# a1q123456/image_stitching

Hardware: AMD Instinct MI355X
Metric: 4K frames stitched/sec (higher is better)
Workload: dtype u8

## Files before the change

### image_stitching_amd/csrc/homography.h

```cpp
#pragma once
#include "common.h"

struct HomoCall {
    const float* src;
    const float* dst;
    uint8_t* mask;
    long long pt_off;
    int n;
    int active;
};

struct HomoResult {
    double H[9];
    int ok;
    int iters;
    int ninl;
    int pad;
};

struct HomoBatch {
    int count = 0;
    long long points = 0;
    int max_iters = 0;
    void* mem = nullptr;
    size_t bytes = 0;
    HomoCall* calls = nullptr;
    HomoResult* results = nullptr;
    void* state = nullptr;
    int* sub_idx = nullptr;
    double* Hc = nullptr;
    int* valid = nullptr;
    int* good = nullptr;
    float* scr = nullptr;
    double* rec = nullptr;
    unsigned* draw_next = nullptr;
    int* draw_idx = nullptr;
    int* fin = nullptr;
};

int homo_batch_reserve(MisContext* ctx, HomoBatch* b, int count, long long points, int max_iters);
int homo_batch_debug_states(MisContext* ctx, const HomoBatch* b, int* out, int cap);
void homo_batch_release(HomoBatch* b);
enum HomoRun {
    HOMO_BOTH_PHASES = 2,
    HOMO_PHASE0_REPLAY = 3,
    HOMO_PHASE1_REPLAY = 6,
    HOMO_TAIL0_MASK = 10,
    HOMO_TAIL0_REFINE = 11,
    HOMO_TAIL1_MASK = 12,
    HOMO_TAIL1_REFINE = 13,
};
struct HomoSync { hipEvent_t rec = nullptr; int rec_pos = 0; };
int homo_batch_run(MisContext* ctx, HomoBatch* b, double thresh, int max_iters, double confidence, HomoRun run = HOMO_BOTH_PHASES,
                   hipStream_t stream = nullptr, const HomoSync* sync = nullptr);
```

### image_stitching_amd/csrc/homography.hip

```cpp
#include "homography.h"
#include "dev_math.h"
#include <algorithm>
#include <mutex>
#include <vector>

namespace {

#ifndef MIS_PHASE0
#define MIS_PHASE0 128
#endif
constexpr int PHASE0 = MIS_PHASE0;
constexpr int RNG_TABLE = 1 << 17;
constexpr int TB = 256;

struct RansacState {
    int mode;
    int n_sub;
    int iter, niters, max_good, done, best_k, result;
    int tail_pending;
    int draw_k, draw_fail;
    long long draw_pos;
};

__device__ __forceinline__ bool jd_mid(int hi_word) { return (((unsigned)hi_word >> 20) & 0x7ffu) - 653u <= 740u; }
__device__ __forceinline__ double jd_div(double n, double d) {
    double r = __builtin_amdgcn_rcp(d);
    double e = __builtin_fma(-d, r, 1.0);
    r = __builtin_fma(r, e, r);
    e = __builtin_fma(-d, r, 1.0);
    r = __builtin_fma(r, e, r);
    const double q = n * r;
    e = __builtin_fma(-d, q, n);
    return __builtin_fma(e, r, q);
}
__device__ __forceinline__ double jd_sqrt_1to2(double x) {
    const double y = __builtin_amdgcn_rsq(x);
    double g = x * y, h = y * 0.5;
    const double r = __builtin_fma(-h, g, 0.5);
    g = __builtin_fma(g, r, g); h = __builtin_fma(h, r, h);
    double d = __builtin_fma(-g, g, x);
    g = __builtin_fma(d, h, g);
    d = __builtin_fma(-g, g, x);
    return __builtin_fma(d, h, g);
}
__device__ __forceinline__ double cv_hypot(double a, double b) {
    a = fabs(a); b = fabs(b);
    if (a > b) { b /= a; return a * sqrt(1 + b * b); }
    if (b > 0) { a /= b; return b * sqrt(1 + a * a); }
    return 0;
}
template <bool LEAN>
__device__ __forceinline__ void jacobi_rotation(double p, double y, double* c_, double* s_, double* t_) {
    double tt, sn, c;
    if (LEAN) {
        const double ap = fabs(p), ay = fabs(y);
        const double big = fmax(ap, ay), q1 = jd_div(fmin(ap, ay), big);
        tt = ay + big * jd_sqrt_1to2(1 + q1 * q1);
        const double q2 = jd_div(ap, tt);
        sn = tt * jd_sqrt_1to2(1 + q2 * q2);
        c = jd_div(tt, sn);
        sn = jd_div(p, sn); tt = jd_div(p, tt) * p;
    } else {
        tt = fabs(y) + cv_hypot(p, y);
        sn = cv_hypot(p, tt);
        c = tt / sn;
// ... 98 lines not shown
    if (d.lds_mod && rel >= 0 && rel < d.lds_n) return (int)d.lds_u[rel];
    return (int)(draw_at(d, pos) % (unsigned)n);
}

__device__ __forceinline__ long long attempt_len(DrawCtx& d, long long pos, int n, int* idx) {
    for (int i = 0; i < 4; i++) {
        int idx_i;
        bool dup;
        do {
            idx_i = draw_mod_at(d, pos++, n);
            dup = false;
            for (int q = 0; q < i; q++) dup |= idx[q] == idx_i;
        } while (dup);
        idx[i] = idx_i;
    }
    return pos;
}
__device__ __forceinline__ bool subset_passes(const float* src, const float* dst, const int* idx) {
    float ms1[8], ms2[8];
    for (int i = 0; i < 4; i++) {
        const float2 ps = reinterpret_cast<const float2*>(src)[idx[i]], pd = reinterpret_cast<const float2*>(dst)[idx[i]];
        ms1[2 * i] = ps.x; ms1[2 * i + 1] = ps.y;
        ms2[2 * i] = pd.x; ms2[2 * i + 1] = pd.y;
    }
    return check_subset(ms1, ms2);
}

__device__ long long attempt_at(DrawCtx& d, long long pos, const float* src, const float* dst, int n, int* idx, bool* pass) {
    float ms1[8], ms2[8];
    for (int i = 0; i < 4; i++) {
        int idx_i;
        bool dup;
        do {
            idx_i = (int)(draw_at(d, pos++) % (unsigned)n);
            dup = false;
            for (int q = 0; q < i; q++) dup |= idx[q] == idx_i;
        } while (dup);
        idx[i] = idx_i;
        const float2 ps = reinterpret_cast<const float2*>(src)[idx_i], pd = reinterpret_cast<const float2*>(dst)[idx_i];
        ms1[2 * i] = ps.x; ms1[2 * i + 1] = ps.y;
        ms2[2 * i] = pd.x; ms2[2 * i + 1] = pd.y;
    }
    *pass = check_subset(ms1, ms2);
    return pos;
}

constexpr int DRAW_CHUNK = 4096;
#ifndef MIS_DRAW_TB
#define MIS_DRAW_TB 1024
#endif
constexpr int DRAW_TB = MIS_DRAW_TB;
constexpr int DRAW_PTS = 2048;
__global__ __launch_bounds__(DRAW_TB) void draw_kernel(const HomoCall* calls, RansacState* states, int* sub_idx, int* draw_idx, const unsigned* U,
                                                  unsigned long long state_T, int max_iters, int phase, int k_hi_arg) {
#if MIS_CHAIN_PRIO
    __builtin_amdgcn_s_setprio(MIS_CHAIN_PRIO);
#endif
    __shared__ unsigned char tab[DRAW_CHUNK];
    __shared__ float2 pts[2 * DRAW_PTS];
    __shared__ long long s_pos;
    __shared__ int s_k, s_attempts, s_more, s_kfirst, s_nacc;
    __shared__ unsigned short acc_o[DRAW_CHUNK / 4];
    __shared__ unsigned short nxtA[DRAW_CHUNK + 1], nxtB[DRAW_CHUNK + 1];
    __shared__ unsigned char reach[DRAW_CHUNK];
    __shared__ unsigned su[DRAW_CHUNK + 128];
    __shared__ int scan[DRAW_TB];
    __shared__ int s_big, s_firstvis, s_lastaccvis;
    __shared__ long long s_endpos;
    const int b = blockIdx.x, t = threadIdx.x;
#ifdef MIS_TAIL_PROF
    const unsigned long long dpk = wall_clock64();
#endif
    const HomoCall c = calls[b];
    RansacState* st = states + b;
    if (phase == 0) {
        if (t == 0) {
            st->mode = (!c.active || c.n < 4) ? 0 : (c.n == 4 ? 1 : 2);
            st->n_sub = 0; st->iter = 0; st->niters = max_iters > 1 ? max_iters : 1; st->max_good = 0; st->done = 0; st->best_k = -1; st->result = 0; st->tail_pending = 0;
            st->draw_k = 0; st->draw_fail = 0; st->draw_pos = 0;
        }
        if (!c.active || c.n <= 4) return;
    } else {
        if (st->mode != 2 || st->done || st->draw_fail) return;
    }
    __syncthreads();
    const int k_hi = min(k_hi_arg, phase == 0 ? max_iters : st->niters);
    if (t == 0) { s_pos = st->draw_pos; s_k = st->draw_k; s_attempts = 0; s_more = s_k < k_hi; }
    __syncthreads();
    DrawCtx d;
    d.U = U; d.state_T = state_T; d.cur_state = state_T; d.cur_pos = RNG_TABLE;
    const float* psrc = c.src;
    const float* pdst = c.dst;
    if (c.n <= DRAW_PTS) {
        for (int i = t; i < c.n; i += DRAW_TB) { pts[i] = reinterpret_cast<const float2*>(c.src)[i]; pts[DRAW_PTS + i] = reinterpret_cast<const float2*>(c.dst)[i]; }
        psrc = reinterpret_cast<const float*>(pts); pdst = reinterpret_cast<const float*>(pts + DRAW_PTS);
        __syncthreads();
    }
    int* didx = draw_idx + (size_t)b * DRAW_CHUNK * 4;
    int* sidx = sub_idx + (size_t)b * max_iters * 4;
    if (phase == 0 && c.n <= 10) {
        const int n = c.n, total = n * (n - 1) * (n - 2) * (n - 3);
        int any = 0;
        for (int q = t; q < total && !any; q += DRAW_TB) {
            int r = q, id[4];
            id[0] = r % n; r /= n;
            int a1 = r % (n - 1); r /= (n - 1);
            int a2 = r % (n - 2); r /= (n - 2);
// ... 129 lines not shown
#ifdef MIS_TAIL_PROF
            dp_last = wall_clock64();
#endif
            continue;
        }
        __syncthreads();
        for (int o = t; o < DRAW_CHUNK; o += DRAW_TB) {
            if ((tab[o] & 0x7f) == 127) continue;
            int idx[4];
            attempt_len(d, base + o, c.n, idx);
            if (subset_passes(psrc, pdst, idx)) tab[o] |= 0x80;
            *reinterpret_cast<int4*>(didx + 4 * o) = make_int4(idx[0], idx[1], idx[2], idx[3]);
        }
        __syncthreads();
        if (t == 0) {
            long long pos = base;
            int k = s_k, attempts = s_attempts, nacc = 0;
            bool fail = false;
            while (k < k_hi && pos < base + DRAW_CHUNK) {
                unsigned char e = tab[pos - base];
                bool pass;
                if ((e & 0x7f) != 127) {
                    pass = (e & 0x80) != 0;
                    if (pass) acc_o[nacc++] = (unsigned short)(pos - base);
                    pos += e & 0x7f;
                } else {
                    int idx[4];
                    pos = attempt_at(d, pos, psrc, pdst, c.n, idx, &pass);
                    if (pass) { acc_o[nacc++] = 0xffff; sidx[4 * k] = idx[0]; sidx[4 * k + 1] = idx[1]; sidx[4 * k + 2] = idx[2]; sidx[4 * k + 3] = idx[3]; }
                }
                attempts++;
                if (pass) { k++; attempts = 0; }
                else if (attempts >= 10000) { fail = true; break; }
            }
            s_kfirst = s_k; s_nacc = nacc;
            s_pos = pos; s_k = k; s_attempts = attempts;
            s_more = !fail && k < k_hi;
            if (!s_more) { st->draw_pos = pos; st->draw_k = k; st->draw_fail = fail; st->n_sub = k; }
        }
        __syncthreads();
        for (int j = t; j < s_nacc; j += DRAW_TB) {
            const unsigned o = acc_o[j];
            if (o != 0xffff) *reinterpret_cast<int4*>(sidx + 4 * (s_kfirst + j)) = *reinterpret_cast<const int4*>(didx + 4 * o);
        }
        __syncthreads();
    }
#ifdef MIS_TAIL_PROF
    if (t == 0 && dp_chunks) {
        const int ph = phase ? 4 : 0;
        atomicAdd(&g_draw_prof[ph], (unsigned long long)dp_chunks); atomicMax(&g_draw_prof[ph + 1], (unsigned long long)dp_chunks);
        atomicMax(&g_draw_prof[ph + 2], wall_clock64() - dp0); atomicAdd(&g_draw_prof[ph + 3], 1ull);
    }
#endif
}

#ifdef MIS_TAIL_PROF
__device__ unsigned long long g_hyp_prof[8];
#endif
#ifndef MIS_HQ_HYPS
#define MIS_HQ_HYPS 64
#endif
constexpr int HQ_HYPS = MIS_HQ_HYPS;
constexpr int HQ_STRIDE = HQ_HYPS + 1;
constexpr int HQ_ELEMS = 127;
struct QSlot {
    double* base;
    __device__ __forceinline__ double& e(int idx) const { return base[idx * HQ_STRIDE]; }
};
__device__ __forceinline__ int hq_T(int r) { return ((r * (17 - r)) >> 1) - r - 1; }
constexpr int HQ_W = 36, HQ_V = 45, HQ_DUMMY = 126;

struct QCand { double a; int pk; };
template <int CTRL>
__device__ __forceinline__ QCand hq_step(const QCand& c) {
    const int hi = __builtin_amdgcn_update_dpp(0, __double2hiint(c.a), CTRL, 0xf, 0xf, false);
    const int lo = __builtin_amdgcn_update_dpp(0, __double2loint(c.a), CTRL, 0xf, 0xf, false);
    const int pk = __builtin_amdgcn_update_dpp(0, c.pk, CTRL, 0xf, 0xf, false);
    const double oa = __hiloint2double(hi, lo);
    const bool take = (c.a < oa) | ((c.a == oa) & (pk < c.pk));
    QCand r;
    r.a = take ? oa : c.a; r.pk = take ? pk : c.pk;
    return r;
}
__device__ __forceinline__ QCand hq_quad_best(QCand c) {
    c = hq_step<0xB1>(c);
    c = hq_step<0x4E>(c);
    return c;
}

__device__ void jacobi9_quad(const QSlot s, const int q) {
    constexpr int n = 9;
    const double eps = DBL_EPSILON;
    int ii[3];
    bool own[3];
#pragma unroll
    for (int j = 0; j < 3; j++) { ii[j] = q + 4 * j; own[j] = ii[j] < n; }
    for (int e = q; e < n * n; e += 4) s.e(HQ_V + e) = (e % (n + 1) == 0) ? 1. : 0.;
    __builtin_amdgcn_fence(__ATOMIC_ACQ_REL, "wavefront");
    int ir[3], ic[3];
    double arv[3], acv[3];
#pragma unroll
    for (int j = 0; j < 3; j++) {
        const int i = ii[j];
        ir[j] = 0; ic[j] = 0; arv[j] = -1.; acv[j] = -1.;
        if (own[j] && i < n - 1) {
            int m = i + 1;
            double mv = fabs(s.e(hq_T(i) + m));
            for (int c = i + 2; c < n; c++) { const double v = fabs(s.e(hq_T(i) + c)); if (mv < v) mv = v, m = c; }
            ir[j] = m; arv[j] = mv;
        }
        if (own[j] && i > 0) {
            int m = 0;
            double mv = fabs(s.e(hq_T(0) + i));
            for (int r = 1; r < i; r++) { const double v = fabs(s.e(hq_T(r) + i)); if (mv < v) mv = v, m = r; }
            ic[j] = m; acv[j] = mv;
// ... 87 lines not shown
            double tw = s.e(HQ_W + m); s.e(HQ_W + m) = s.e(HQ_W + k); s.e(HQ_W + k) = tw;
            for (int i = 0; i < n; i++) { double tv = s.e(HQ_V + n * m + i); s.e(HQ_V + n * m + i) = s.e(HQ_V + n * k + i); s.e(HQ_V + n * k + i) = tv; }
        }
        __builtin_amdgcn_fence(__ATOMIC_ACQ_REL, "wavefront");
    }
}

__device__ int dlt4_quad(const float* M, const float* m, const QSlot s, const int q, double* H) {
    const int count = 4;
    double cMx = 0, cMy = 0, cmx = 0, cmy = 0, sMx = 0, sMy = 0, smx = 0, smy = 0;
    for (int i = 0; i < count; i++) { cmx += m[2 * i]; cmy += m[2 * i + 1]; cMx += M[2 * i]; cMy += M[2 * i + 1]; }
    cmx /= count; cmy /= count; cMx /= count; cMy /= count;
    for (int i = 0; i < count; i++) {
        smx += fabs(m[2 * i] - cmx); smy += fabs(m[2 * i + 1] - cmy);
        sMx += fabs(M[2 * i] - cMx); sMy += fabs(M[2 * i + 1] - cMy);
    }
    if (fabs(smx) < DBL_EPSILON || fabs(smy) < DBL_EPSILON || fabs(sMx) < DBL_EPSILON || fabs(sMy) < DBL_EPSILON) return 0;
    smx = count / smx; smy = count / smy; sMx = count / sMx; sMy = count / sMy;
    double LtL[45];
#pragma unroll
    for (int e = 0; e < 45; e++) LtL[e] = 0;
#pragma unroll
    for (int i = 0; i < count; i++) {
        const double x = (m[2 * i] - cmx) * smx, y = (m[2 * i + 1] - cmy) * smy;
        const double X = (M[2 * i] - cMx) * sMx, Y = (M[2 * i + 1] - cMy) * sMy;
        const double Lx[9] = {X, Y, 1, 0, 0, 0, -x * X, -x * Y, -x};
        const double Ly[9] = {0, 0, 0, X, Y, 1, -y * X, -y * Y, -y};
        int e = 0;
#pragma unroll
        for (int j = 0; j < 9; j++)
#pragma unroll
            for (int k = j; k < 9; k++, e++) LtL[e] += Lx[j] * Lx[k] + Ly[j] * Ly[k];
    }
    {
        int e = 0;
#pragma unroll
        for (int j = 0; j < 9; j++)
#pragma unroll
            for (int k = j; k < 9; k++, e++) {
                if ((e & 3) != q) continue;
                if (k == j) s.e(HQ_W + j) = LtL[e];
                else s.e(hq_T(j) + k) = LtL[e];
            }
    }
    __builtin_amdgcn_fence(__ATOMIC_ACQ_REL, "wavefront");
    jacobi9_quad(s, q);
    double H0[9];
    for (int i = 0; i < 9; i++) H0[i] = s.e(HQ_V + 72 + i);
    const double nrm[8] = {cmx, cmy, cMx, cMy, smx, smy, sMx, sMy};
    dlt_denormalise(H0, nrm, H);
    return 1;
}

__global__ __launch_bounds__(4 * HQ_HYPS) void hyp_quad_kernel(const HomoCall* calls, const RansacState* states, const int* sub_idx, double* Hc, int* valid, int lo,
                                                               int max_iters) {
#if MIS_CHAIN_PRIO
    __builtin_amdgcn_s_setprio(MIS_CHAIN_PRIO);
#endif
    extern __shared__ double sl[];
    const int b = blockIdx.y, t = threadIdx.x, h = t >> 2, q = t & 3;
    const RansacState st = states[b];
    if (st.mode != 2 || st.done) return;
    const int limit = min(st.n_sub, st.niters);
    const int k = lo + blockIdx.x * HQ_HYPS + h;
    if (k >= limit) return;
    const HomoCall c = calls[b];
    const int* id = sub_idx + ((size_t)b * max_iters + k) * 4;
    float ms1[8], ms2[8];
#pragma unroll
    for (int i = 0; i < 4; i++) {
        int qq = id[i];
        ms1[2 * i] = c.src[2 * qq]; ms1[2 * i + 1] = c.src[2 * qq + 1];
        ms2[2 * i] = c.dst[2 * qq]; ms2[2 * i + 1] = c.dst[2 * qq + 1];
    }
    double H[9];
    const QSlot s{sl + h};
    const int ok = dlt4_quad(ms1, ms2, s, q, H);
    if (q == 0) {
        if (ok) {
            double* o = Hc + ((size_t)b * max_iters + k) * 9;
#pragma unroll
            for (int i = 0; i < 9; i++) o[i] = H[i];
        }
        valid[(size_t)b * max_iters + k] = ok;
    }
}

__global__ __launch_bounds__(256) void hyp_count_kernel(const HomoCall* calls, const RansacState* states, const double* Hc, const int* valid, int* good, int lo,
                                                        int max_iters, float thr) {
    const int b = blockIdx.y, lane = threadIdx.x & 63;
    const RansacState st = states[b];
    if (st.mode != 2 || st.done) return;
    const int limit = min(st.n_sub, st.niters);
    const int k = lo + blockIdx.x * 4 + (int)(threadIdx.x >> 6);
    if (k >= limit) return;
    const size_t e = (size_t)b * max_iters + k;
    int cnt = 0;
    if (valid[e]) {
        const HomoCall c = calls[b];
        float Hf[9];
#pragma unroll
        for (int i = 0; i < 9; i++) Hf[i] = (float)Hc[e * 9 + i];
        for (int i0 = 0; i0 < c.n; i0 += 64) {
            const int i = i0 + lane;
            const int f = i < c.n ? is_inlier(Hf, c.src[2 * i], c.src[2 * i + 1], c.dst[2 * i], c.dst[2 * i + 1], thr) : 0;
            cnt += __popcll(__ballot(f));
        }
    }
    if (lane == 0) good[e] = cnt;
}

#ifdef MIS_TAIL_PROF
__device__ unsigned long long g_jac_prof[8];
#ifdef MIS_JAC_PROF
#define JP_T(v) const unsigned long long v = __builtin_readcyclecounter()
#define JP_ADD(i, a, b) do { if (threadIdx.x == 0) atomicAdd(&g_jac_prof[i], (b) - (a)); } while (0)
#else
#define JP_T(v)
#define JP_ADD(i, a, b)
#endif
__device__ unsigned long long g_tail_log[6 * 1024];
__device__ unsigned g_tail_log_n;
__device__ unsigned long long g_tail_prof[12];
#define PROF_T0(v) unsigned long long v = wall_clock64()
#define PROF_ADD(i, v) do { if (threadIdx.x == 0) atomicAdd(&g_tail_prof[i], wall_clock64() - (v)); } while (0)
#define PROF_INC(i, n) do { if (threadIdx.x == 0) atomicAdd(&g_tail_prof[i], (unsigned long long)(n)); } while (0)
#else
#define PROF_T0(v)
#define PROF_ADD(i, v)
#define PROF_INC(i, n)
#define JP_T(v)
#define JP_ADD(i, a, b)
#endif
#ifndef MIS_PS_PTS
#define MIS_PS_PTS 32
#endif
constexpr int PS_PTS = MIS_PS_PTS;
constexpr int PS_TERMS = 42;
constexpr int PS_PITCH = 43;
constexpr int PS_STAGE = PS_PTS * PS_PITCH;
constexpr size_t TAIL_DYN_LDS = sizeof(double) * 2 * PS_STAGE;
struct TailShared {
    double A[81], V[81], W[9];
    double best[9], nrm[8];
    double lm[8 + 8 + 64 + 64 + 8 + 8 + 8 + 8];
    float Hf[9];
    int indR[9], indC[9];
    int np, go;
    int bad;
    double chunk[TB * 10];
    int staged;
#ifdef MIS_TAIL_PROF
    int prof_rot, prof_lm;
#endif
};
__device__ __forceinline__ float4 tail_load_point(const float* s1, const float* d1, int i) {
    const float2 dd = reinterpret_cast<const float2*>(d1)[i], ss = reinterpret_cast<const float2*>(s1)[i];
    return make_float4(dd.x, dd.y, ss.x, ss.y);
}
__device__ __forceinline__ void lds_barrier() { mis_lds_barrier(); }

__device__ __forceinline__ void wave_sync() {
// ... 520 lines not shown
        }
        __syncthreads();
        if (sc[6] != 0.) {
            if (t < 64) S.A[t] = A[t];
            __syncthreads();
            jacobi_eigen_coop<8>(S);
            if (t == 0) {
                double thrw = 0;
                for (int i = 0; i < 8; i++) thrw += S.W[i];
                thrw *= DBL_EPSILON * 2;
                for (int e = 0; e < 64; e++) Ap[e] = 0;
                for (int i = 0; i < 8; i++) {
                    double wi = S.W[i];
                    if (fabs(wi) <= thrw) continue;
                    wi = 1 / wi;
                    for (int r = 0; r < 8; r++)
                        for (int c = 0; c < 8; c++) Ap[r * 8 + c] = Ap[r * 8 + c] + S.V[i * 8 + r] * (S.V[i * 8 + c] * wi);
                }
                double maxval = DBL_EPSILON;
                for (int i = 0; i < 8; i++) { double a = fabs(Ap[i * 8 + i]); if (a > maxval) maxval = a; }
                double lambda = 1. / maxval, nu = sc[7] * 0.5;
                sc[5] = lambda;
                sc[4] = lambda * nu;
            }
            __syncthreads();
        }
        if (t == 0) {
            double Sv = sc[0], Sd = sc[1];
            sc[3] = Sd < Sv ? 1. : 0.;
            if (Sd < Sv) { sc[0] = Sd; for (int i = 0; i < 8; i++) x[i] = xd[i]; }
        }
        __syncthreads();
        if (sc[3] != 0.) normal_eq(x, true);
        iter++;
        PROF_INC(3, 1);
#ifdef MIS_TAIL_PROF
        if (t == 0) S.prof_lm++;
#endif
        double dmax = 0;
        for (int i = 0; i < 8; i++) { double a = fabs(d[i]); if (a > dmax) dmax = a; }
        bool proceed = iter < 10 && dmax >= (double)FLT_EPSILON && sc[2] >= (double)FLT_EPSILON;
        __syncthreads();
        if (!proceed) break;
    }
    if (t < 8) S.best[t] = x[t];
    __syncthreads();
}

#ifndef MIS_TAIL_WAVES
#define MIS_TAIL_WAVES 3
#endif
__global__ __launch_bounds__(TB) __attribute__((amdgpu_waves_per_eu(MIS_TAIL_WAVES, 8))) void scan_tail_kernel(const HomoCall* calls, RansacState* states, const double* Hc, const int* valid, const int* good,
                                                       float* scr_all, double* rec_all, HomoResult* results, int lo, int hi, int max_iters,
                                                       double confidence, float thr, int* fin, int part, int want, int staged) {
#if MIS_CHAIN_PRIO
    __builtin_amdgcn_s_setprio(MIS_CHAIN_PRIO);
#endif
#ifdef MIS_TAIL_PROF
    const unsigned long long wg_in = wall_clock64();
    if (part == 4 && want == 0 && threadIdx.x == 0) atomicMin(&g_tail_prof[8], wg_in);
#endif
    __shared__ TailShared S;
    __shared__ int s_done_now;
    if (threadIdx.x == 0) { S.staged = staged; S.bad = 0; }
    if (staged)
        for (int i = threadIdx.x; i < 2 * PS_PTS; i += TB) tail_dyn[i * PS_PITCH + PS_TERMS] = 0.;
    __syncthreads();
    __shared__ int wcnt[TB / 64];
    __shared__ int s_base;
    const int b = blockIdx.x, t = threadIdx.x;
    const HomoCall c = calls[b];
    RansacState* st = states + b;
    HomoResult* res = results + b;
    const int n = c.n;
    float* s1 = scr_all + 4 * c.pt_off;
    float* d1 = s1 + 2 * (size_t)(n > 0 ? n : 0);
    double* rec = rec_all + 10 * c.pt_off;
    if (part >= 3) {
        if (st->tail_pending != (part == 4 ? 2 : 1) || fin[b] != want) return;
        __syncthreads();
    } else {
    if (st->done) return;
    const int mode = st->mode;
    if (t == 0) s_done_now = 0;
    __syncthreads();
    if (mode == 0) {
        for (int i = t; c.mask && c.active && i < n; i += TB) c.mask[i] = 0;
        if (t == 0) { res->ok = 0; res->iters = 0; res->ninl = 0; st->done = 1; fin[b] = lo == 0 ? 0 : 1; }
        return;
    }
    if (mode == 1) {
        if (t == 0) for (int i = 0; i < 9; i++) S.best[i] = 0;
        __syncthreads();
        dlt_coop(S, c.src, c.dst, 4, t < 4 ? tail_load_point(c.src, c.dst, t) : make_float4(0.f, 0.f, 0.f, 0.f), rec);
        const int ok = S.go;
        for (int i = t; c.mask && i < n; i += TB) c.mask[i] = ok ? 1 : 0;
        if (t == 0) { res->ok = ok; res->iters = 0; res->ninl = ok ? 4 : 0; if (ok) for (int i = 0; i < 9; i++) res->H[i] = S.best[i]; st->done = 1; fin[b] = lo == 0 ? 0 : 1; }
        return;
    }
    {
#ifdef MIS_TAIL_PROF
        const unsigned long long rp0 = wall_clock64();
#endif
        const int nsub = st->n_sub, kmax = min(hi, nsub), cnt = max(min(kmax - lo, st->niters - st->iter), 0);
        int* gl = reinterpret_cast<int*>(S.chunk);
        int* segmax = gl + 4096;
        const bool staged = cnt <= 4096;
// ... 79 lines not shown
#ifdef MIS_TAIL_PROF
    if (t == 0) { S.prof_rot = 0; S.prof_lm = 0; }
#endif
    if (np > 0) {
        const float4 pt0 = t < np ? tail_load_point(s1, d1, t) : make_float4(0.f, 0.f, 0.f, 0.f);
        dlt_coop(S, s1, d1, np, pt0, rec);
        PROF_ADD(4, pt);
        lm_refine_coop(S, s1, d1, np, pt0, rec);
    }
    PROF_ADD(5, pt);
    PROF_INC(6, 1);
#ifdef MIS_TAIL_PROF
    if (t == 0) atomicMax(&g_tail_prof[7], wall_clock64() - pt);
    if (t == 0) {
        const unsigned k = atomicAdd(&g_tail_log_n, 1u);
        if (k < 1024) { unsigned long long* e = g_tail_log + 6 * k; e[0] = np; e[1] = S.prof_lm; e[2] = S.prof_rot; e[3] = wall_clock64() - pt; e[4] = part * 10 + want; e[5] = pt; }
    }
    if (part == 4 && want == 0 && t == 0) { const unsigned long long o = wall_clock64(); atomicMax(&g_tail_prof[9], o); atomicMax(&g_tail_prof[10], o - wg_in); atomicAdd(&g_tail_prof[11], 1ull); }
#endif
    if (t == 0) { for (int i = 0; i < 9; i++) res->H[i] = S.best[i]; res->ninl = np; if (part == 4) st->tail_pending = 0; }
}

struct RngTable {
    unsigned* U = nullptr;
    unsigned long long state_T = 0;
};
std::mutex g_rng_mutex;
RngTable g_rng[64];

int rng_table(MisContext* ctx, RngTable* out) {
    std::lock_guard<std::mutex> lock(g_rng_mutex);
    RngTable& r = g_rng[ctx->device & 63];
    if (!r.U) {
        std::vector<unsigned> h(RNG_TABLE);
        unsigned long long st = ~0ull;
        for (int i = 0; i < RNG_TABLE; i++) {
            st = (unsigned long long)(unsigned)st * 4164903690u + (unsigned)(st >> 32);
            h[i] = (unsigned)st;
        }
        MIS_HIP(ctx, hipMalloc((void**)&r.U, sizeof(unsigned) * RNG_TABLE));
        MIS_HIP(ctx, hipMemcpy(r.U, h.data(), sizeof(unsigned) * RNG_TABLE, hipMemcpyHostToDevice));
        r.state_T = st;
    }
    *out = r;
    return MIS_OK;
}

}

int homo_batch_reserve(MisContext* ctx, HomoBatch* b, int count, long long points, int max_iters) {
    count = std::max(count, 1); points = std::max(points, 1ll); max_iters = std::max(max_iters, 1);
    size_t off = 0;
    auto carve = [&](size_t bytes) { size_t o = off; off += mis_align_up(bytes, 256); return o; };
    size_t o_calls = carve(sizeof(HomoCall) * count), o_res = carve(sizeof(HomoResult) * count), o_state = carve(sizeof(RansacState) * count);
    size_t o_sub = carve(sizeof(int) * 4 * (size_t)count * max_iters), o_hc = carve(sizeof(double) * 9 * (size_t)count * max_iters);
    size_t o_valid = carve(sizeof(int) * (size_t)count * max_iters), o_good = carve(sizeof(int) * (size_t)count * max_iters);
    size_t o_scr = carve(sizeof(float) * 4 * (size_t)points), o_rec = carve(sizeof(double) * 10 * (size_t)points);
    size_t o_dn = carve(256), o_di = carve(sizeof(int) * 4 * (size_t)count * DRAW_CHUNK), o_fin = carve(sizeof(int) * (size_t)count);
    if (off > b->bytes) {
        if (b->mem) { MIS_HIP(ctx, hipStreamSynchronize(ctx->stream)); MIS_HIP(ctx, hipFree(b->mem)); b->mem = nullptr; b->bytes = 0; }
        MIS_HIP(ctx, hipMalloc(&b->mem, off));
        b->bytes = off;
    }
    uint8_t* m = (uint8_t*)b->mem;
    b->calls = (HomoCall*)(m + o_calls); b->results = (HomoResult*)(m + o_res); b->state = m + o_state;
    b->sub_idx = (int*)(m + o_sub); b->Hc = (double*)(m + o_hc); b->valid = (int*)(m + o_valid); b->good = (int*)(m + o_good);
    b->scr = (float*)(m + o_scr); b->rec = (double*)(m + o_rec); b->draw_next = (unsigned*)(m + o_dn); b->draw_idx = (int*)(m + o_di); b->fin = (int*)(m + o_fin);
    b->count = count; b->points = points; b->max_iters = max_iters;
    return MIS_OK;
}

#ifdef MIS_TAIL_PROF
extern "C" int mis_debug_tail_prof(unsigned long long* out, int reset) {
    hipDeviceSynchronize();
    hipMemcpyFromSymbol(out, HIP_SYMBOL(g_tail_prof), sizeof(unsigned long long) * 12);
    if (reset) { unsigned long long z[12] = {0}; z[8] = ~0ull; hipMemcpyToSymbol(HIP_SYMBOL(g_tail_prof), z, sizeof(z)); }
    return 0;
}
extern "C" int mis_debug_tail_log(unsigned long long* out, int cap, int reset) {
    unsigned n = 0;
    if (hipMemcpyFromSymbol(&n, HIP_SYMBOL(g_tail_log_n), sizeof(n)) != hipSuccess) return -1;
    if (n > 1024) n = 1024;
    if ((int)n > cap) n = cap;
    if (n && hipMemcpyFromSymbol(out, HIP_SYMBOL(g_tail_log), sizeof(unsigned long long) * 6 * n) != hipSuccess) return -1;
    if (reset) { unsigned z = 0; if (hipMemcpyToSymbol(HIP_SYMBOL(g_tail_log_n), &z, sizeof(z)) != hipSuccess) return -1; }
    return (int)n;
}
extern "C" int mis_debug_draw_prof(unsigned long long* out, int reset) {
    hipDeviceSynchronize();
    hipMemcpyFromSymbol(out, HIP_SYMBOL(g_draw_prof), sizeof(unsigned long long) * 12);
    if (reset) { unsigned long long z[12] = {0}; hipMemcpyToSymbol(HIP_SYMBOL(g_draw_prof), z, sizeof(z)); }
    return 0;
}
extern "C" int mis_debug_hyp_prof(unsigned long long* out, int reset) {
    hipDeviceSynchronize();
    hipMemcpyFromSymbol(out, HIP_SYMBOL(g_hyp_prof), sizeof(unsigned long long) * 8);
    if (reset) { unsigned long long z[8] = {0}; hipMemcpyToSymbol(HIP_SYMBOL(g_hyp_prof), z, sizeof(z)); }
    return 0;
}
extern "C" int mis_debug_jac_prof(unsigned long long* out, int reset) {
    hipDeviceSynchronize();
    hipMemcpyFromSymbol(out, HIP_SYMBOL(g_jac_prof), sizeof(unsigned long long) * 8);
    if (reset) { unsigned long long z[8] = {0}; hipMemcpyToSymbol(HIP_SYMBOL(g_jac_prof), z, sizeof(z)); }
    return 0;
}
#endif

int homo_batch_debug_states(MisContext* ctx, const HomoBatch* b, int* out, int cap) {
    const int n = std::min(cap, b->count);
    std::vector<RansacState> st(n);
    std::vector<HomoCall> calls(n);
    MIS_HIP(ctx, hipStreamSynchronize(ctx->stream));
    MIS_HIP(ctx, hipMemcpy(st.data(), b->state, sizeof(RansacState) * n, hipMemcpyDeviceToHost));
    MIS_HIP(ctx, hipMemcpy(calls.data(), b->calls, sizeof(HomoCall) * n, hipMemcpyDeviceToHost));
    for (int i = 0; i < n; i++) {
        int* o = out + 8 * i;
        o[0] = calls[i].n; o[1] = st[i].mode; o[2] = st[i].n_sub; o[3] = st[i].iter; o[4] = st[i].niters; o[5] = st[i].draw_fail; o[6] = st[i].done; o[7] = st[i].max_good;
    }
    return n;
}

void homo_batch_release(HomoBatch* b) {
    if (b->mem) hipFree(b->mem);
    b->mem = nullptr; b->bytes = 0;
}

int homo_batch_run(MisContext* ctx, HomoBatch* b, double thresh, int max_iters, double confidence, HomoRun run, hipStream_t stream, const HomoSync* sync) {
    const HomoSync none;
    const HomoSync& sy = sync ? *sync : none;
    MIS_CHECK(ctx, max_iters >= 1 && max_iters <= b->max_iters, MIS_E_INVALID, "max_iters %d outside the reserved range", max_iters);
    MIS_CHECK(ctx, confidence > 0 && confidence < 1, MIS_E_INVALID, "confidence must be in (0,1)");
    RngTable rt;
    int rc = rng_table(ctx, &rt);
    if (rc != MIS_OK) return rc;
    if (thresh <= 0) thresh = 3;
    const float thr = (float)(thresh * thresh);
    hipStream_t st = stream ? stream : ctx->stream;
    static bool attr_set[64] = {false};
    const size_t hq_lds = sizeof(double) * HQ_ELEMS * HQ_STRIDE;
    if (!attr_set[ctx->device & 63]) {
        MIS_HIP(ctx, hipFuncSetAttribute((const void*)hyp_quad_kernel, hipFuncAttributeMaxDynamicSharedMemorySize, (int)hq_lds));
        attr_set[ctx->device & 63] = true;
    }
    RansacState* states = (RansacState*)b->state;
    const int p0 = std::min(PHASE0, max_iters);
    static const bool plain = getenv("MIS_TAIL_PLAIN") != nullptr && atoi(getenv("MIS_TAIL_PLAIN")) != 0;
    auto tail_staged = [&](int part) { return (part == 1 || part == 3 || plain) ? 0 : 1; };
    auto tail_lds = [&](int part) { return tail_staged(part) ? TAIL_DYN_LDS : (size_t)0; };
    const int replay_part = run == HOMO_BOTH_PHASES ? 0 : 1;
    if (run == HOMO_BOTH_PHASES || run == HOMO_PHASE0_REPLAY) {
        MIS_HIP(ctx, hipMemsetAsync(b->fin, 0xff, sizeof(int) * (size_t)b->count, st));
        hipLaunchKernelGGL(draw_kernel, dim3(b->count), dim3(DRAW_TB), 0, st, b->calls, states, b->sub_idx, b->draw_idx, rt.U, rt.state_T, max_iters, 0, p0);
        if (sy.rec && sy.rec_pos == 2) MIS_HIP(ctx, hipEventRecord(sy.rec, st));
        hipLaunchKernelGGL(hyp_quad_kernel, dim3((p0 + HQ_HYPS - 1) / HQ_HYPS, b->count), dim3(4 * HQ_HYPS), hq_lds, st, b->calls, states, b->sub_idx, b->Hc, b->valid, 0, max_iters);
        hipLaunchKernelGGL(hyp_count_kernel, dim3((p0 + 3) / 4, b->count), dim3(256), 0, st, b->calls, states, (const double*)b->Hc, (const int*)b->valid, b->good, 0, max_iters, thr);
        hipLaunchKernelGGL(scan_tail_kernel, dim3(b->count), dim3(TB), tail_lds(replay_part), st, b->calls, states, b->Hc, b->valid, b->good, b->scr, b->rec, b->results, 0, p0,
                           max_iters, confidence, thr, b->fin, replay_part, 0, tail_staged(replay_part));
    }
    if (run >= HOMO_TAIL0_MASK) {
        const int want = (run - HOMO_TAIL0_MASK) >> 1, part = 3 + ((run - HOMO_TAIL0_MASK) & 1);
        hipLaunchKernelGGL(scan_tail_kernel, dim3(b->count), dim3(TB), tail_lds(part), st, b->calls, states, b->Hc, b->valid, b->good, b->scr, b->rec, b->results, 0, p0,
                           max_iters, confidence, thr, b->fin, part, want, tail_staged(part));
    }
    if ((run == HOMO_BOTH_PHASES || run == HOMO_PHASE1_REPLAY) && max_iters > p0) {
        hipLaunchKernelGGL(draw_kernel, dim3(b->count), dim3(DRAW_TB), 0, st, b->calls, states, b->sub_idx, b->draw_idx, rt.U, rt.state_T, max_iters, 1, max_iters);
        if (sy.rec && sy.rec_pos == 0) MIS_HIP(ctx, hipEventRecord(sy.rec, st));
        hipLaunchKernelGGL(hyp_quad_kernel, dim3((max_iters - p0 + HQ_HYPS - 1) / HQ_HYPS, b->count), dim3(4 * HQ_HYPS), hq_lds, st, b->calls, states, b->sub_idx, b->Hc, b->valid, p0, max_iters);
        hipLaunchKernelGGL(hyp_count_kernel, dim3((max_iters - p0 + 3) / 4, b->count), dim3(256), 0, st, b->calls, states, (const double*)b->Hc, (const int*)b->valid, b->good, p0,
                           max_iters, thr);
        hipLaunchKernelGGL(scan_tail_kernel, dim3(b->count), dim3(TB), tail_lds(replay_part), st, b->calls, states, b->Hc, b->valid, b->good, b->scr, b->rec, b->results, p0,
                           max_iters, max_iters, confidence, thr, b->fin, replay_part, 0, tail_staged(replay_part));
    }
    MIS_HIP(ctx, hipGetLastError());
    return MIS_OK;
}
```

Baseline: 3252.

## Compact RANSAC hypothesis work into a list and run persistent ticketed kernels

The draw kernel now appends live (batch, k-offset) work-list entries through an atomic counter. The hypothesis solve and count kernels become persistent grids sized per CU that pull tickets from this list, so dead or finished batches no longer launch empty blocks. The count kernel also scores four hypotheses per wave against each loaded point, with a 4-way point unroll, so point loads are reused across hypotheses. The scan tail kernel resets the counters for the next phase. The cost is extra atomics, a dependency on counter reset ordering, and more registers in the count kernel.

```diff
diff --git a/image_stitching_amd/csrc/homography.h b/image_stitching_amd/csrc/homography.h
--- a/image_stitching_amd/csrc/homography.h
+++ b/image_stitching_amd/csrc/homography.h
@@ -36,6 +36,8 @@
     unsigned* draw_next = nullptr;
     int* draw_idx = nullptr;
     int* fin = nullptr;
+    int2* work = nullptr;
+    unsigned* work_ctr = nullptr;
 };
 
 int homo_batch_reserve(MisContext* ctx, HomoBatch* b, int count, long long points, int max_iters);
diff --git a/image_stitching_amd/csrc/homography.hip b/image_stitching_amd/csrc/homography.hip
--- a/image_stitching_amd/csrc/homography.hip
+++ b/image_stitching_amd/csrc/homography.hip
@@ -11,6 +11,10 @@
 #endif
 constexpr int PHASE0 = MIS_PHASE0;
 constexpr int RNG_TABLE = 1 << 17;
+#ifndef MIS_HQ_HYPS
+#define MIS_HQ_HYPS 64
+#endif
+constexpr int HQ_HYPS = MIS_HQ_HYPS;
 constexpr int TB = 256;
 
 struct RansacState {
@@ -215,7 +219,7 @@
 constexpr int DRAW_TB = MIS_DRAW_TB;
 constexpr int DRAW_PTS = 2048;
 __global__ __launch_bounds__(DRAW_TB) void draw_kernel(const HomoCall* calls, RansacState* states, int* sub_idx, int* draw_idx, const unsigned* U,
-                                                  unsigned long long state_T, int max_iters, int phase, int k_hi_arg) {
+                                                  unsigned long long state_T, int max_iters, int phase, int k_hi_arg, int2* work, unsigned* work_ctr) {
 #if MIS_CHAIN_PRIO
     __builtin_amdgcn_s_setprio(MIS_CHAIN_PRIO);
 #endif
@@ -451,15 +455,19 @@
         atomicMax(&g_draw_prof[ph + 2], wall_clock64() - dp0); atomicAdd(&g_draw_prof[ph + 3], 1ull);
     }
 #endif
+    if (t == 0) {
+        const int lo = phase == 0 ? 0 : min(PHASE0, max_iters), hi = min(st->n_sub, st->niters);
+        if (st->mode == 2 && !st->done && hi > lo) {
+            const int nb = (hi - lo + HQ_HYPS - 1) / HQ_HYPS;
+            const unsigned at = atomicAdd(work_ctr, (unsigned)nb);
+            for (int i = 0; i < nb; i++) work[at + i] = make_int2(b, lo + i * HQ_HYPS);
+        }
+    }
 }
 
 #ifdef MIS_TAIL_PROF
 __device__ unsigned long long g_hyp_prof[8];
 #endif
-#ifndef MIS_HQ_HYPS
-#define MIS_HQ_HYPS 64
-#endif
-constexpr int HQ_HYPS = MIS_HQ_HYPS;
 constexpr int HQ_STRIDE = HQ_HYPS + 1;
 constexpr int HQ_ELEMS = 127;
 struct QSlot {
@@ -653,62 +661,100 @@
     return 1;
 }
 
-__global__ __launch_bounds__(4 * HQ_HYPS) void hyp_quad_kernel(const HomoCall* calls, const RansacState* states, const int* sub_idx, double* Hc, int* valid, int lo,
-                                                               int max_iters) {
+constexpr int HQ_WG_PER_CU = 2;
+constexpr int HC_WG_PER_CU = 4;
+constexpr int HC_HYPS = 4;
+enum { WL_N = 0, WL_SOLVE = 1, WL_CTRS = 2 };
+static_assert(HQ_HYPS % 16 == 0 && HQ_HYPS % HC_HYPS == 0, "a work-list entry splits into whole solve and count tickets");
+__device__ __forceinline__ unsigned first_ticket() { return __builtin_amdgcn_readfirstlane(blockIdx.x * (blockDim.x >> 6) + (threadIdx.x >> 6)); }
+__device__ __forceinline__ unsigned next_ticket(unsigned* ctr, unsigned tickets) {
+    const unsigned waves = gridDim.x * (blockDim.x >> 6);
+    if (tickets <= waves) return tickets;
+    return waves + __builtin_amdgcn_readfirstlane(atomicAdd(ctr, (threadIdx.x & 63) == 0 ? 1u : 0u));
+}
+
+__global__ __launch_bounds__(4 * HQ_HYPS) void hyp_quad_kernel(const HomoCall* calls, const RansacState* states, const int* sub_idx, double* Hc, int* valid,
+                                                               int max_iters, const int2* work, unsigned* work_ctr) {
 #if MIS_CHAIN_PRIO
     __builtin_amdgcn_s_setprio(MIS_CHAIN_PRIO);
 #endif
     extern __shared__ double sl[];
-    const int b = blockIdx.y, t = threadIdx.x, h = t >> 2, q = t & 3;
-    const RansacState st = states[b];
-    if (st.mode != 2 || st.done) return;
-    const int limit = min(st.n_sub, st.niters);
-    const int k = lo + blockIdx.x * HQ_HYPS + h;
-    if (k >= limit) return;
-    const HomoCall c = calls[b];
-    const int* id = sub_idx + ((size_t)b * max_iters + k) * 4;
-    float ms1[8], ms2[8];
-#pragma unroll
-    for (int i = 0; i < 4; i++) {
-        int qq = id[i];
-        ms1[2 * i] = c.src[2 * qq]; ms1[2 * i + 1] = c.src[2 * qq + 1];
-        ms2[2 * i] = c.dst[2 * qq]; ms2[2 * i + 1] = c.dst[2 * qq + 1];
-    }
-    double H[9];
+    const int lane = threadIdx.x & 63, q = lane & 3;
+    const int h = threadIdx.x >> 2;
+    const unsigned tickets = work_ctr[WL_N] * (HQ_HYPS / 16);
     const QSlot s{sl + h};
-    const int ok = dlt4_quad(ms1, ms2, s, q, H);
-    if (q == 0) {
-        if (ok) {
-            double* o = Hc + ((size_t)b * max_iters + k) * 9;
-#pragma unroll
-            for (int i = 0; i < 9; i++) o[i] = H[i];
-        }
-        valid[(size_t)b * max_iters + k] = ok;
-    }
-}
-
-__global__ __launch_bounds__(256) void hyp_count_kernel(const HomoCall* calls, const RansacState* states, const double* Hc, const int* valid, int* good, int lo,
-                                                        int max_iters, float thr) {
-    const int b = blockIdx.y, lane = threadIdx.x & 63;
-    const RansacState st = states[b];
-    if (st.mode != 2 || st.done) return;
-    const int limit = min(st.n_sub, st.niters);
-    const int k = lo + blockIdx.x * 4 + (int)(threadIdx.x >> 6);
-    if (k >= limit) return;
-    const size_t e = (size_t)b * max_iters + k;
-    int cnt = 0;
-    if (valid[e]) {
+    for (unsigned tk = first_ticket(); tk < tickets; tk = next_ticket(work_ctr + WL_SOLVE, tickets)) {
+        const int2 w = work[tk / (HQ_HYPS / 16)];
+        const int b = w.x;
+        const RansacState& st = states[b];
+        const int limit = min(st.n_sub, st.niters);
+        const int k = w.y + (int)(tk % (HQ_HYPS / 16)) * 16 + (lane >> 2);
+        if (k < limit) {
+            const HomoCall c = calls[b];
+            const int* id = sub_idx + ((size_t)b * max_iters + k) * 4;
+            float ms1[8], ms2[8];
+#pragma unroll
+            for (int i = 0; i < 4; i++) {
+                int qq = id[i];
+                ms1[2 * i] = c.src[2 * qq]; ms1[2 * i + 1] = c.src[2 * qq + 1];
+                ms2[2 * i] = c.dst[2 * qq]; ms2[2 * i + 1] = c.dst[2 * qq + 1];
+            }
+            double H[9];
+            const int ok = dlt4_quad(ms1, ms2, s, q, H);
+            if (ok) {
+                double* o = Hc + ((size_t)b * max_iters + k) * 9;
+#pragma unroll
+                for (int i = 0; i < 9; i++) o[i] = H[i];
+            }
+            valid[(size_t)b * max_iters + k] = ok;
+        }
+    }
+}
+
+constexpr int HC_UNROLL = 4;
+__global__ __launch_bounds__(256) void hyp_count_kernel(const HomoCall* calls, const RansacState* states, const double* Hc, const int* valid, int* good,
+                                                        int max_iters, float thr, const int2* work, const unsigned* work_ctr) {
+    const int lane = threadIdx.x & 63;
+    const unsigned tickets = work_ctr[WL_N] * (HQ_HYPS / HC_HYPS), waves = gridDim.x * (blockDim.x >> 6);
+    for (unsigned tk = first_ticket(); tk < tickets; tk += waves) {
+        const int2 w = work[tk / (HQ_HYPS / HC_HYPS)];
+        const int b = w.x;
+        const RansacState& st = states[b];
+        const int limit = min(st.n_sub, st.niters);
+        const int k0 = w.y + (int)(tk % (HQ_HYPS / HC_HYPS)) * HC_HYPS;
+        if (k0 >= limit) continue;
+        const size_t e0 = (size_t)b * max_iters + k0;
+        float Hf[HC_HYPS][9];
+        bool use[HC_HYPS];
+        int cnt[HC_HYPS];
+#pragma unroll
+        for (int j = 0; j < HC_HYPS; j++) {
+            use[j] = k0 + j < limit && valid[e0 + j];
+            cnt[j] = 0;
+#pragma unroll
+            for (int i = 0; i < 9; i++) Hf[j][i] = use[j] ? (float)Hc[(e0 + j) * 9 + i] : 0.f;
+        }
         const HomoCall c = calls[b];
-        float Hf[9];
-#pragma unroll
-        for (int i = 0; i < 9; i++) Hf[i] = (float)Hc[e * 9 + i];
-        for (int i0 = 0; i0 < c.n; i0 += 64) {
-            const int i = i0 + lane;
-            const int f = i < c.n ? is_inlier(Hf, c.src[2 * i], c.src[2 * i + 1], c.dst[2 * i], c.dst[2 * i + 1], thr) : 0;
-            cnt += __popcll(__ballot(f));
-        }
-    }
-    if (lane == 0) good[e] = cnt;
+        const float2* src = reinterpret_cast<const float2*>(c.src);
+        const float2* dst = reinterpret_cast<const float2*>(c.dst);
+        for (int i0 = 0; i0 < c.n; i0 += 64 * HC_UNROLL) {
+            float2 M[HC_UNROLL], m[HC_UNROLL];
+            bool in[HC_UNROLL];
+#pragma unroll
+            for (int u = 0; u < HC_UNROLL; u++) {
+                const int i = i0 + 64 * u + lane;
+                in[u] = i < c.n;
+                M[u] = src[min(i, c.n - 1)]; m[u] = dst[min(i, c.n - 1)];
+            }
+#pragma unroll
+            for (int u = 0; u < HC_UNROLL; u++)
+#pragma unroll
+                for (int j = 0; j < HC_HYPS; j++)
+                    if (use[j]) cnt[j] += __popcll(__ballot(in[u] && is_inlier(Hf[j], M[u].x, M[u].y, m[u].x, m[u].y, thr)));
+        }
+#pragma unroll
+        for (int j = 0; j < HC_HYPS; j++) if (k0 + j < limit) good[e0 + j] = cnt[j];
+    }
 }
 
 #ifdef MIS_TAIL_PROF
@@ -1335,7 +1381,8 @@
 #endif
 __global__ __launch_bounds__(TB) __attribute__((amdgpu_waves_per_eu(MIS_TAIL_WAVES, 8))) void scan_tail_kernel(const HomoCall* calls, RansacState* states, const double* Hc, const int* valid, const int* good,
                                                        float* scr_all, double* rec_all, HomoResult* results, int lo, int hi, int max_iters,
-                                                       double confidence, float thr, int* fin, int part, int want, int staged) {
+                                                       double confidence, float thr, int* fin, int part, int want, int staged, unsigned* work_ctr) {
+    if (work_ctr && blockIdx.x == 0 && threadIdx.x < WL_CTRS) work_ctr[threadIdx.x] = 0;
 #if MIS_CHAIN_PRIO
     __builtin_amdgcn_s_setprio(MIS_CHAIN_PRIO);
 #endif
@@ -1521,20 +1568,25 @@
     count = std::max(count, 1); points = std::max(points, 1ll); max_iters = std::max(max_iters, 1);
     size_t off = 0;
     auto carve = [&](size_t bytes) { size_t o = off; off += mis_align_up(bytes, 256); return o; };
+    const size_t o_wctr = carve(sizeof(unsigned) * WL_CTRS);
     size_t o_calls = carve(sizeof(HomoCall) * count), o_res = carve(sizeof(HomoResult) * count), o_state = carve(sizeof(RansacState) * count);
     size_t o_sub = carve(sizeof(int) * 4 * (size_t)count * max_iters), o_hc = carve(sizeof(double) * 9 * (size_t)count * max_iters);
     size_t o_valid = carve(sizeof(int) * (size_t)count * max_iters), o_good = carve(sizeof(int) * (size_t)count * max_iters);
     size_t o_scr = carve(sizeof(float) * 4 * (size_t)points), o_rec = carve(sizeof(double) * 10 * (size_t)points);
     size_t o_dn = carve(256), o_di = carve(sizeof(int) * 4 * (size_t)count * DRAW_CHUNK), o_fin = carve(sizeof(int) * (size_t)count);
+    const size_t o_work = carve(sizeof(int2) * (size_t)count * ((max_iters + HQ_HYPS - 1) / HQ_HYPS));
     if (off > b->bytes) {
         if (b->mem) { MIS_HIP(ctx, hipStreamSynchronize(ctx->stream)); MIS_HIP(ctx, hipFree(b->mem)); b->mem = nullptr; b->bytes = 0; }
         MIS_HIP(ctx, hipMalloc(&b->mem, off));
         b->bytes = off;
+        MIS_HIP(ctx, hipMemsetAsync((uint8_t*)b->mem + o_wctr, 0, sizeof(unsigned) * WL_CTRS, ctx->stream));
+        MIS_HIP(ctx, hipStreamSynchronize(ctx->stream));
     }
     uint8_t* m = (uint8_t*)b->mem;
     b->calls = (HomoCall*)(m + o_calls); b->results = (HomoResult*)(m + o_res); b->state = m + o_state;
     b->sub_idx = (int*)(m + o_sub); b->Hc = (double*)(m + o_hc); b->valid = (int*)(m + o_valid); b->good = (int*)(m + o_good);
     b->scr = (float*)(m + o_scr); b->rec = (double*)(m + o_rec); b->draw_next = (unsigned*)(m + o_dn); b->draw_idx = (int*)(m + o_di); b->fin = (int*)(m + o_fin);
+    b->work = (int2*)(m + o_work); b->work_ctr = (unsigned*)(m + o_wctr);
     b->count = count; b->points = points; b->max_iters = max_iters;
     return MIS_OK;
 }
@@ -1617,28 +1669,34 @@
     auto tail_staged = [&](int part) { return (part == 1 || part == 3 || plain) ? 0 : 1; };
     auto tail_lds = [&](int part) { return tail_staged(part) ? TAIL_DYN_LDS : (size_t)0; };
     const int replay_part = run == HOMO_BOTH_PHASES ? 0 : 1;
+    const int ncu = std::max(ctx->num_cu, 1);
+    auto hypotheses = [&]() {
+        hipLaunchKernelGGL(hyp_quad_kernel, dim3(HQ_WG_PER_CU * ncu), dim3(4 * HQ_HYPS), hq_lds, st, b->calls, states, b->sub_idx, b->Hc, b->valid, max_iters,
+                           (const int2*)b->work, b->work_ctr);
+        hipLaunchKernelGGL(hyp_count_kernel, dim3(HC_WG_PER_CU * ncu), dim3(256), 0, st, b->calls, states, (const double*)b->Hc, (const int*)b->valid, b->good,
+                           max_iters, thr, (const int2*)b->work, b->work_ctr);
+    };
     if (run == HOMO_BOTH_PHASES || run == HOMO_PHASE0_REPLAY) {
         MIS_HIP(ctx, hipMemsetAsync(b->fin, 0xff, sizeof(int) * (size_t)b->count, st));
-        hipLaunchKernelGGL(draw_kernel, dim3(b->count), dim3(DRAW_TB), 0, st, b->calls, states, b->sub_idx, b->draw_idx, rt.U, rt.state_T, max_iters, 0, p0);
+        hipLaunchKernelGGL(draw_kernel, dim3(b->count), dim3(DRAW_TB), 0, st, b->calls, states, b->sub_idx, b->draw_idx, rt.U, rt.state_T, max_iters, 0, p0, b->work,
+                           b->work_ctr);
         if (sy.rec && sy.rec_pos == 2) MIS_HIP(ctx, hipEventRecord(sy.rec, st));
-        hipLaunchKernelGGL(hyp_quad_kernel, dim3((p0 + HQ_HYPS - 1) / HQ_HYPS, b->count), dim3(4 * HQ_HYPS), hq_lds, st, b->calls, states, b->sub_idx, b->Hc, b->valid, 0, max_iters);
-        hipLaunchKernelGGL(hyp_count_kernel, dim3((p0 + 3) / 4, b->count), dim3(256), 0, st, b->calls, states, (const double*)b->Hc, (const int*)b->valid, b->good, 0, max_iters, thr);
+        hypotheses();
         hipLaunchKernelGGL(scan_tail_kernel, dim3(b->count), dim3(TB), tail_lds(replay_part), st, b->calls, states, b->Hc, b->valid, b->good, b->scr, b->rec, b->results, 0, p0,
-                           max_iters, confidence, thr, b->fin, replay_part, 0, tail_staged(replay_part));
+                           max_iters, confidence, thr, b->fin, replay_part, 0, tail_staged(replay_part), b->work_ctr);
     }
     if (run >= HOMO_TAIL0_MASK) {
         const int want = (run - HOMO_TAIL0_MASK) >> 1, part = 3 + ((run - HOMO_TAIL0_MASK) & 1);
         hipLaunchKernelGGL(scan_tail_kernel, dim3(b->count), dim3(TB), tail_lds(part), st, b->calls, states, b->Hc, b->valid, b->good, b->scr, b->rec, b->results, 0, p0,
-                           max_iters, confidence, thr, b->fin, part, want, tail_staged(part));
+                           max_iters, confidence, thr, b->fin, part, want, tail_staged(part), nullptr);
     }
     if ((run == HOMO_BOTH_PHASES || run == HOMO_PHASE1_REPLAY) && max_iters > p0) {
-        hipLaunchKernelGGL(draw_kernel, dim3(b->count), dim3(DRAW_TB), 0, st, b->calls, states, b->sub_idx, b->draw_idx, rt.U, rt.state_T, max_iters, 1, max_iters);
+        hipLaunchKernelGGL(draw_kernel, dim3(b->count), dim3(DRAW_TB), 0, st, b->calls, states, b->sub_idx, b->draw_idx, rt.U, rt.state_T, max_iters, 1, max_iters,
+                           b->work, b->work_ctr);
         if (sy.rec && sy.rec_pos == 0) MIS_HIP(ctx, hipEventRecord(sy.rec, st));
-        hipLaunchKernelGGL(hyp_quad_kernel, dim3((max_iters - p0 + HQ_HYPS - 1) / HQ_HYPS, b->count), dim3(4 * HQ_HYPS), hq_lds, st, b->calls, states, b->sub_idx, b->Hc, b->valid, p0, max_iters);
-        hipLaunchKernelGGL(hyp_count_kernel, dim3((max_iters - p0 + 3) / 4, b->count), dim3(256), 0, st, b->calls, states, (const double*)b->Hc, (const int*)b->valid, b->good, p0,
-                           max_iters, thr);
+        hypotheses();
         hipLaunchKernelGGL(scan_tail_kernel, dim3(b->count), dim3(TB), tail_lds(replay_part), st, b->calls, states, b->Hc, b->valid, b->good, b->scr, b->rec, b->results, p0,
-                           max_iters, max_iters, confidence, thr, b->fin, replay_part, 0, tail_staged(replay_part));
+                           max_iters, max_iters, confidence, thr, b->fin, replay_part, 0, tail_staged(replay_part), b->work_ctr);
     }
     MIS_HIP(ctx, hipGetLastError());
     return MIS_OK;
```

New measurement: 3333 (median of 6 runs). 1.03x the previous value.
